# HTDerekLiu/surface_multigrid_code

Measured on AMD Instinct MI355X. Metric: V-cycles/sec + fine-level SpMV GB/s (% HBM peak), 1M-vert mesh fp64, higher is better.
Workload: dtype f64; 1 GPU; C3: bunny_15K_init x3 midpoint subdivision, 1011330 verts, 5 levels, M_bary+0.01(-L), fp64; n_verts=1011330, nnz=7079298, levels=5, smoother=gs, rhs_columns_per_gpu=1, parallelism=single GPU

## Files before the change

surface_multigrid_code_amd/csrc/smg_cycle.cpp:

```cpp
#include <hip/hip_runtime.h>

#include <algorithm>
#include <chrono>
#include <cmath>
#include <cstdarg>
#include <cstdio>
#include <cstdlib>
#include <cstring>
#include <functional>
#include <memory>
#include <numeric>
#include <string>
#include <thread>
#include <vector>

#include "smg_internal.hpp"

using namespace smg;


static hipError_t ensure_map(DevBuf<int>& d, const std::vector<int>& host)
{
    if (d.n == host.size() && (d.p || host.empty())) return hipSuccess;
    return d.upload(host);
// ... 360 lines not shown
    }
    if (k > h->kcap32) {
        drop_graphs(h);
        for (int lv = 0; lv < L; lv++) {
            Level& Lv = h->lv[lv];
            const size_t rows = (lv == L - 1) ? (size_t)h->nc_pad : (size_t)Lv.n;
            HIPCHK(Lv.b32.alloc(rows * k));
            HIPCHK(Lv.u32.alloc(rows * k));
            HIPCHK(hipMemsetAsync(Lv.b32.p, 0, rows * k * sizeof(float), h->stream));
            HIPCHK(hipMemsetAsync(Lv.u32.p, 0, rows * k * sizeof(float), h->stream));
            if (lv < L - 1) HIPCHK(Lv.r32.alloc(rows * k));
            Lv.t32.release(); Lv.d32.release();
        }
        h->kcap32 = k;
    }
    for (int lv = 0; lv < L - 1; lv++) {
        Level& Lv = h->lv[lv];
        if (level_is_jacobi(h, lv) && Lv.t32.n < (size_t)Lv.n * h->kcap32) {
            drop_graphs(h);
            HIPCHK(Lv.t32.alloc((size_t)Lv.n * h->kcap32));
            HIPCHK(hipMemsetAsync(Lv.t32.p, 0, (size_t)Lv.n * h->kcap32 * sizeof(float), h->stream));
        }
        if (level_kind(h, lv) == LV_CHEBY && Lv.d32.n < (size_t)Lv.n * h->kcap32) {
            drop_graphs(h);
            HIPCHK(Lv.d32.alloc((size_t)Lv.n * h->kcap32));
            HIPCHK(hipMemsetAsync(Lv.d32.p, 0, (size_t)Lv.n * h->kcap32 * sizeof(float), h->stream));
        }
    }
    if (h->coarse_schur) {
        const size_t need = (size_t)h->sch.view.ns_pad * std::max(h->kcap32, 1);
        if (h->sch.g32.n < need || h->sch.xs32.n < need) {
            drop_graphs(h);
            HIPCHK(h->sch.g32.alloc(need));
            HIPCHK(h->sch.xs32.alloc(need));
            HIPCHK(hipMemsetAsync(h->sch.g32.p, 0, need * sizeof(float), h->stream));
            HIPCHK(hipMemsetAsync(h->sch.xs32.p, 0, need * sizeof(float), h->stream));
        }
        h->sch.view.g32 = h->sch.g32.p; h->sch.view.xs32 = h->sch.xs32.p;
    }
    return SMG_OK;
}

int smg::level_kind(const smg_hierarchy* h, int lv)
{
    if (lv < 0 || lv >= h->n_levels - 1) return LV_GS;
    switch (h->smoother) {
        case SMG_SMOOTH_JACOBI: return LV_JACOBI;
        case SMG_SMOOTH_HYBRID: return h->lv[lv].n <= h->jacobi_max_rows ? LV_JACOBI : LV_GS;
        case SMG_SMOOTH_CHEBYSHEV: return LV_CHEBY;
        case SMG_SMOOTH_HYBRID_CHEBYSHEV: return h->lv[lv].n <= h->jacobi_max_rows ? LV_CHEBY : LV_GS;
    }
    return LV_GS;
}

struct ChebyCoef { double c1, c2; };
static void cheby_coefs(double lam, double frac, int degree, std::vector<ChebyCoef>& out)
{
    out.resize((size_t)std::max(degree, 0));
    const double lmax = lam, lmin = lam * frac;
    const double theta = (lmax + lmin) / 2.0, delta = (lmax - lmin) / 2.0;
    const double sigma = theta / delta;
    double rho = 1.0 / sigma;
    for (int s = 0; s < degree; s++) {
        if (s == 0) { out[s].c1 = 0.0; out[s].c2 = 1.0 / theta; }
        else {
            const double rho_new = 1.0 / (2.0 * sigma - rho);
            out[s].c1 = rho_new * rho;
            out[s].c2 = 2.0 * rho_new / delta;
            rho = rho_new;
        }
    }
}

template <typename T> struct Prec;
static inline int coarse_cols(const smg_hierarchy* h, int k) { return (h->coarse_cols > 0 && h->coarse_cols < k) ? h->coarse_cols : k; }

template <> struct Prec<double> {
    static double* b(Level& L) { return L.b.p; }
    static double* u(Level& L) { return L.u.p; }
    static double* r(Level& L) { return L.r.p; }
    static double* t(Level& L) { return L.t.p; }
    static double* d(Level& L) { return L.d.p; }
    static void set_d(FirstColour& fc, Level& L) { fc.d = L.d.p; }
    static const SellDev& A(Level& L) { return L.dA.view; }
    static const SellDev& G(Level& L) { return L.gs_on_transpose ? L.dAT.view : L.dA.view; }
    static const SellDev& P(Level& L) { return L.dP.view; }
    static const SellDev& PT(Level& L) { return L.dPT.view; }
    static bool has_vals(const SellDev& V) { return V.val != nullptr; }
    static hipError_t sell(SellMode m, const SellDev& V, int s0, int s1, const double* x, const double* bb, double* y, int k, const Ctrl* ctrl,
                           hipStream_t st, double* zero_rows = nullptr, const FirstColour* first = nullptr, double omega = 1.0)
    { return launch_sell(m, V, s0, s1, x, bb, y, k, ctrl, nullptr, nullptr, st, zero_rows, first, omega); }
    static hipError_t coarse(smg_hierarchy* h, Level& L, int k, const Ctrl* ctrl)
    {
        if (h->union_m > 0) return launch_blockdiag_gemv_add(h->un.view, h->d_Ainv.p, h->nc, L.b.p, L.u.p, k, ctrl, h->stream);
        if (h->coarse_sparse) return launch_sparse_coarse_solve(h->c_view, L.b.p, L.u.p, k, ctrl, h->stream);
        if (h->coarse_schur) return launch_schur_solve(h->sch.view, L.b.p, L.u.p, k, ctrl, h->stream);
        return launch_dense_gemv_add(h->d_Ainv.p, h->nc, h->nc_pad, L.b.p, L.u.p, coarse_cols(h, k), k, ctrl, h->stream, h->d_sympart.p);
    }
    static hipError_t opA(smg_hierarchy* h, Level& L, bool smoother_image, SellMode m, int s0, int s1, const double* x, const double* bb, double* y, int k,
                          const Ctrl* ctrl, const FirstColour* fc = nullptr, double omega = 1.0)
    {
        if (h->bs == 3) {
            const Bsr3Dev& V = (smoother_image && L.gs_on_transpose) ? L.bAT.view : L.bA.view;
            return launch_bsr3(m, V, s0, s1 < 0 ? V.n_slices : s1, x, bb, y, k, ctrl, nullptr, nullptr, h->stream, omega, fc ? fc->c1 : 0.0, fc ? fc->d : nullptr);
        }
        const SellDev& V = smoother_image ? G(L) : A(L);
        return sell(m, V, s0, s1 < 0 ? V.n_slices : s1, x, bb, y, k, ctrl, h->stream, nullptr, fc, omega);
    }
};
template <> struct Prec<float> {
    static float* b(Level& L) { return L.b32.p; }
    static float* u(Level& L) { return L.u32.p; }
    static float* r(Level& L) { return L.r32.p; }
    static float* t(Level& L) { return L.t32.p; }
    static float* d(Level& L) { return L.d32.p; }
    static void set_d(FirstColour& fc, Level& L) { fc.df = L.d32.p; }
    static const SellDev& A(Level& L) { return L.dA32; }
    static const SellDev& G(Level& L) { return L.gs_on_transpose ? L.dAT32 : L.dA32; }
    static const SellDev& P(Level& L) { return L.dP32; }
    static const SellDev& PT(Level& L) { return L.dPT32; }
    static bool has_vals(const SellDev& V) { return V.valf != nullptr; }
    static hipError_t sell(SellMode m, const SellDev& V, int s0, int s1, const float* x, const float* bb, float* y, int k, const Ctrl* ctrl,
                           hipStream_t st, float* zero_rows = nullptr, const FirstColour* first = nullptr, double omega = 1.0)
    { return launch_sell_f32(m, V, s0, s1, x, bb, y, k, ctrl, st, zero_rows, first, omega); }
    static hipError_t coarse(smg_hierarchy* h, Level& L, int k, const Ctrl* ctrl)
    {
        if (h->coarse_schur) return launch_schur_solve_f32(h->sch.view, L.b32.p, L.u32.p, k, ctrl, h->stream);
        return launch_dense_gemv_add_f32(h->d_Ainv32.p, h->nc, h->nc_pad, L.b32.p, L.u32.p, coarse_cols(h, k), k, ctrl, h->stream, (float*)h->d_sympart.p);
    }
    static hipError_t opA(smg_hierarchy* h, Level& L, bool smoother_image, SellMode m, int s0, int s1, const float* x, const float* bb, float* y, int k,
                          const Ctrl* ctrl, const FirstColour* fc = nullptr, double omega = 1.0)
    {
        if (h->bs == 3) {
            const Bsr3Dev& V = (smoother_image && L.gs_on_transpose) ? L.bAT.view : L.bA.view;
            return launch_bsr3_f32(m, V, s0, s1 < 0 ? V.n_slices : s1, x, bb, y, k, ctrl, h->stream, omega, fc ? fc->c1 : 0.0, fc ? fc->df : nullptr);
        }
        const SellDev& V = smoother_image ? G(L) : A(L);
        return sell(m, V, s0, s1 < 0 ? V.n_slices : s1, x, bb, y, k, ctrl, h->stream, nullptr, fc, omega);
    }
};

static const std::vector<int>& colour_slices(const smg_hierarchy* h, const Level& Lv)
{
    if (h->bs == 3) return (Lv.gs_on_transpose ? Lv.bAT : Lv.bA).color_slice_ptr;
    return (Lv.gs_on_transpose ? Lv.dAT : Lv.dA).color_slice_ptr;
}

enum { FIRST_NONE = 0,
       FIRST_LAUNCH = 1,
       FIRST_SWEEP = 2 };

template <typename T>
static int enqueue_gs(smg_hierarchy* h, int lv, const T* b, T* u, int k, int iters, const Ctrl* ctrl, int first = FIRST_NONE, T* t = nullptr)
{
    Level& Lv = h->lv[lv];
    ProfGuard pg(h, "MG: relaxation");
    if (std::is_same<T, double>::value && first == FIRST_NONE) {
        if (const WgsBuf* W = wgs_plan(h, lv, k)) {
            for (int it = 0; it < iters; it++)
                for (size_t c = 0; c + 1 < W->color_ptr.size(); c++)
                    HIPCHK(launch_wgs(W->view, W->color_ptr[c], W->color_ptr[c + 1], (const double*)b, (double*)u, k, ctrl, h->stream));
            return SMG_OK;
        }
        if (const BgsBuf* Q = bgs_plan(h, lv, k)) {
            for (int it = 0; it < iters; it++)
                for (size_t c = 0; c + 1 < Q->color_ptr.size(); c++)
                    HIPCHK(launch_bgs(Q->view, Q->color_ptr[c], Q->color_ptr[c + 1], (const double*)b, (double*)u, k, ctrl, h->stream));
            return SMG_OK;
        }
    }
    const std::vector<int>& cs = colour_slices(h, Lv);
    for (int it = first == FIRST_SWEEP ? 1 : 0; it < iters; it++)
        for (size_t c = (it == 0 && first == FIRST_LAUNCH) ? 1 : 0; c + 1 < cs.size(); c++) {
            if (it == 1 && first == FIRST_SWEEP) HIPCHK(Prec<T>::sell(SELL_GS_OOP, Prec<T>::G(Lv), cs[c], cs[c + 1], t, b, u, k, ctrl, h->stream));
            else HIPCHK(Prec<T>::opA(h, Lv, true, SELL_GS, cs[c], cs[c + 1], u, b, u, k, ctrl));
        }
    return SMG_OK;
}

static int enqueue_gs_tiled(smg_hierarchy* h, int lv, const TiledDev& plan, const double* b, double* const buf[2], int* cur, int k, const Ctrl* ctrl)
{
    ProfGuard pg(h, "MG: relaxation");
    HIPCHK(launch_tiled_gs(plan, buf[*cur], b, buf[1 - *cur], k, ctrl, h->stream));
    *cur ^= 1;
    return SMG_OK;
}
template <typename T> static const TiledDev* tiled_for(const smg_hierarchy*, Level&, int, int, int) { return nullptr; }
template <> const TiledDev* tiled_for<double>(const smg_hierarchy* h, Level& Lv, int lv, int k, int sweeps)
{
    const TiledDev* p = tiled_plan(h, lv, k, sweeps);
    return (p && Lv.t.p) ? p : nullptr;
}
template <typename T> static int enqueue_gs_tiled_t(smg_hierarchy*, int, const TiledDev&, const T*, T* const*, int*, int, const Ctrl*) { return SMG_ERR_INVALID; }
template <> int enqueue_gs_tiled_t<double>(smg_hierarchy* h, int lv, const TiledDev& plan, const double* b, double* const* buf, int* cur, int k, const Ctrl* ctrl)
{
    double* const two[2] = {buf[0], buf[1]};
    return enqueue_gs_tiled(h, lv, plan, b, two, cur, k, ctrl);
}

template <typename T>
static int enqueue_jacobi(smg_hierarchy* h, int lv, const T* b, T* const buf[2], int* cur, int k, int iters, const Ctrl* ctrl)
{
    Level& Lv = h->lv[lv];
    ProfGuard pg(h, "MG: relaxation");
    for (int it = 0; it < iters; it++) {
        HIPCHK(Prec<T>::opA(h, Lv, true, SELL_JACOBI, 0, -1, buf[*cur], b, buf[1 - *cur], k, ctrl, nullptr, h->omega));
        *cur ^= 1;
    }
    return SMG_OK;
}

template <typename T>
static int enqueue_cheby(smg_hierarchy* h, int lv, const T* b, T* const buf[2], int* cur, int k, int iters, const Ctrl* ctrl, bool first_done = false)
{
    if (iters <= 0) return SMG_OK;
    Level& Lv = h->lv[lv];
    ProfGuard pg(h, "MG: relaxation");
    std::vector<ChebyCoef> cf;
    cheby_coefs(Lv.lam, h->cheby_fraction, iters + 1, cf);
    for (int s = first_done ? 1 : 0; s <= iters; s++) {
        FirstColour fc;
        Prec<T>::set_d(fc, Lv);
        fc.c1 = cf[s].c1;
        HIPCHK(Prec<T>::opA(h, Lv, true, SELL_CHEBY, 0, -1, buf[*cur], b, buf[1 - *cur], k, ctrl, &fc, cf[s].c2));
        *cur ^= 1;
    }
    return SMG_OK;
}

static bool fuse_first_colour() { static const int on = env_int("SMG_FUSE_FIRST", 1); return on != 0; }

template <typename T>
static int enqueue_vcycle_t(smg_hierarchy* h, int lv, int k, int pre, int post, const Ctrl* ctrl, int first = FIRST_NONE)
{
    const bool first_done = first != FIRST_NONE;
    const int L = h->n_levels;
    Level& Lv = h->lv[lv];
    if (lv == L - 1) {
        ProfGuard pg(h, "MG: coarse solve");
        HIPCHK(Prec<T>::coarse(h, Lv, k, ctrl));
        return SMG_OK;
    }
    Level& Lc = h->lv[lv + 1];
    const int kind = level_kind(h, lv);
    const bool jac = kind != LV_GS;
    T* const buf[2] = {Prec<T>::u(Lv), Prec<T>::t(Lv)};
    int cur = 0;
    const TiledDev* tl_pre = (kind == LV_GS && pre > 0 && first != FIRST_SWEEP) ? tiled_for<T>(h, Lv, lv, k, pre) : nullptr;
    const TiledDev* tl_post = (kind == LV_GS && post > 0) ? tiled_for<T>(h, Lv, lv, k, post) : nullptr;
    int rc;
    if (kind == LV_JACOBI) {
        if (first_done) cur = 1;
        rc = enqueue_jacobi<T>(h, lv, Prec<T>::b(Lv), buf, &cur, k, pre - (first_done ? 1 : 0), ctrl);
    } else if (kind == LV_CHEBY) {
        if (first_done) cur = 1;
        rc = enqueue_cheby<T>(h, lv, Prec<T>::b(Lv), buf, &cur, k, pre, ctrl, first_done);
    } else if (tl_pre) rc = enqueue_gs_tiled_t<T>(h, lv, *tl_pre, Prec<T>::b(Lv), buf, &cur, k, ctrl);
    else rc = enqueue_gs<T>(h, lv, Prec<T>::b(Lv), buf[0], k, pre, ctrl, first, buf[1]);
    if (rc) return rc;
    {
        ProfGuard pg(h, "MG: residual");
        HIPCHK(Prec<T>::opA(h, Lv, false, SELL_RESID, 0, -1, buf[cur], Prec<T>::b(Lv), Prec<T>::r(Lv), k, ctrl));
    }
    const SellBuf& Gc = Lc.gs_on_transpose ? Lc.dAT : Lc.dA;
    const int kind_c = level_kind(h, lv + 1);
    const bool jac_c = kind_c != LV_GS;
    const bool tiled_c = level_kind(h, lv + 1) == LV_GS && pre > 0 && tiled_for<T>(h, Lc, lv + 1, k, pre) != nullptr;
    const bool fuse = h->bs == 1 && !tiled_c && !(std::is_same<T, double>::value && (bgs_plan(h, lv + 1, k) || wgs_plan(h, lv + 1, k))) && fuse_first_colour() && lv + 1 < L - 1 && pre > 0 && Prec<T>::has_vals(Prec<T>::G(Lc)) && (jac_c ? Gc.n_all > 0 : Gc.n_first > 0);
    const int kt = k * h->bs;
    {
        ProfGuard pg(h, "MG: restrict");
        FirstColour fc;
        if (fuse) {
            fc.diag_slot = Gc.diag_slot.p; fc.n_first = jac_c ? Gc.n_all : Gc.n_first;
            fc.val = Prec<T>::G(Lc).val; fc.valf = Prec<T>::G(Lc).valf;
            fc.jacobi = kind_c == LV_CHEBY ? 2 : (jac_c ? 1 : 0); fc.omega = h->omega;
            if (kind_c == LV_CHEBY) {
                std::vector<ChebyCoef> cf;
                cheby_coefs(Lc.lam, h->cheby_fraction, 1, cf);
                fc.omega = cf[0].c2;
                Prec<T>::set_d(fc, Lc);
            }
        }
        T* init = (fuse && jac_c) ? Prec<T>::t(Lc) : Prec<T>::u(Lc);
        HIPCHK(Prec<T>::sell(SELL_AX, Prec<T>::PT(Lc), 0, Prec<T>::PT(Lc).n_slices, Prec<T>::r(Lv), nullptr, Prec<T>::b(Lc), kt, ctrl, h->stream, init,
                             fuse ? &fc : nullptr));
    }
    rc = enqueue_vcycle_t<T>(h, lv + 1, k, pre, post, ctrl, fuse ? FIRST_LAUNCH : FIRST_NONE);
    if (rc) return rc;
    {
        ProfGuard pg(h, "MG: prolong");
        int dst = cur;
        const int flips = tl_post ? 1 : kind == LV_CHEBY ? (post > 0 ? post + 1 : 0) : post;
        if ((jac || tl_post) && ((cur + flips) & 1)) dst = 1 - cur;
        if (!jac && !tl_post && cur == 1) dst = 0;
        HIPCHK(Prec<T>::sell(SELL_ADD, Prec<T>::P(Lc), 0, Prec<T>::P(Lc).n_slices, Prec<T>::u(Lc), buf[cur], buf[dst], kt, ctrl, h->stream));
        cur = dst;
    }
    if (kind == LV_CHEBY) return enqueue_cheby<T>(h, lv, Prec<T>::b(Lv), buf, &cur, k, post, ctrl);
    if (jac) return enqueue_jacobi<T>(h, lv, Prec<T>::b(Lv), buf, &cur, k, post, ctrl);
    if (tl_post) return enqueue_gs_tiled_t<T>(h, lv, *tl_post, Prec<T>::b(Lv), buf, &cur, k, ctrl);
    return enqueue_gs<T>(h, lv, Prec<T>::b(Lv), buf[0], k, post, ctrl);
}

static int enqueue_vcycle(smg_hierarchy* h, int lv, int k, int pre, int post, const Ctrl* ctrl, int first = FIRST_NONE)
{
    return enqueue_vcycle_t<double>(h, lv, k, pre, post, ctrl, first);
}
static int enqueue_vcycle32(smg_hierarchy* h, int lv, int k, int pre, int post, const Ctrl* ctrl)
{
    return enqueue_vcycle_t<float>(h, lv, k, pre, post, ctrl);
}

static int enqueue_relax(smg_hierarchy* h, int lv, const double* b, double* u, int k, int iters, const Ctrl* ctrl)
{
    if (!level_is_jacobi(h, lv)) {
        Level& Lg = h->lv[lv];
        if (const TiledDev* tl = tiled_for<double>(h, Lg, lv, k, iters)) {
            double* const two[2] = {u, Lg.t.p};
            int c2 = 0;
            int rc = enqueue_gs_tiled(h, lv, *tl, b, two, &c2, k, ctrl);
            if (rc) return rc;
            HIPCHK(hipMemcpyAsync(u, Lg.t.p, (size_t)Lg.n * k * sizeof(double), hipMemcpyDeviceToDevice, h->stream));
            return SMG_OK;
        }
        return enqueue_gs<double>(h, lv, b, u, k, iters, ctrl);
    }
    Level& Lv = h->lv[lv];
    double* const buf[2] = {u, Lv.t.p};
    int cur = 0;
    int rc = level_kind(h, lv) == LV_CHEBY ? enqueue_cheby<double>(h, lv, b, buf, &cur, k, iters, ctrl)
                                           : enqueue_jacobi<double>(h, lv, b, buf, &cur, k, iters, ctrl);
    if (rc) return rc;
    if (cur == 1) HIPCHK(hipMemcpyAsync(u, Lv.t.p, (size_t)Lv.n * k * sizeof(double), hipMemcpyDeviceToDevice, h->stream));
    return SMG_OK;
}

static bool head_fusable(smg_hierarchy* h, int k)
{
    static const int on = env_int("SMG_FUSE_HEAD", 1);
    if (!on || h->precision != 0 || h->n_levels < 2 || h->prof_on || h->bs != 1 || h->union_m > 0) return false;
    Level& L0 = h->lv[0];
    if (L0.gs_on_transpose) return false;
    if (bgs_plan(h, 0, k) || wgs_plan(h, 0, k)) return false;
    if (level_kind(h, 0) == LV_GS && tiled_plan(h, 0, k, h->pre) && L0.t.p) return false;
// ... 900 lines not shown
```

surface_multigrid_code_amd/csrc/smg_device.hip:

```cpp
#include <hip/hip_runtime.h>

#include <cstdlib>
#include <type_traits>

#include "smg_device.hpp"
#include "smg_device_inl.hpp"
#include "smg_gj_inl.hpp"

namespace smg {


__device__ int g_never_done = 0;
const int* never_done()
{
    static const int* p = nullptr;
    if (!p) { void* q = nullptr; if (hipGetSymbolAddress(&q, HIP_SYMBOL(g_never_done)) == hipSuccess) p = (const int*)q; }
    return p;
}


template <typename T> struct CoarseInit { T* u; const T* gs_val; const int* diag_slot; int n_first; int jacobi; T omega; T* d; T c1; };

template <int MODE, int KB, typename T, int W0C = -1, int WPB = 4>
__global__ __launch_bounds__(64 * WPB) void k_sell(const int* a_col, const T* a_val, const int* a_order, const int* a_slice_off, int a_stride,
                                              int a_w_lo, int s_begin, int s_end, int n_blocks, int use_order, const T* x,
                                              const int* a_slice_row, const int* a_slice_w, const T* b, T* y, int ld, const int* done,
                                              double* partials, CoarseInit<T> z)
{
    struct { const int *slice_row, *slice_off, *slice_w, *order, *col; int stride, w_lo; } A = {a_slice_row, a_slice_off, a_slice_w, a_order,
                                                                                               a_col, a_stride, a_w_lo};
    constexpr int C = 64;
    const int lane = threadIdx.x & 63;
    const int wave = threadIdx.x >> 6;
    constexpr int wpb = WPB;
    constexpr bool GS = sell_is_gs(MODE), OOP = sell_is_oop(MODE), JAC = sell_is_jacobi(MODE), CHEB = sell_is_cheby(MODE), HEAD = sell_is_head(MODE);
    int bid;
    if (GS && n_blocks < 0) { if (blockIdx.x & 7) return; bid = blockIdx.x >> 3; }
    else bid = xcd_remap(blockIdx.x, n_blocks);
    const int ls = __builtin_amdgcn_readfirstlane(s_begin + bid * wpb + wave);
    double ss = 0.0;
    int stop = 0;
    if (ls < s_end) {
        const int s = (!GS && use_order) ? A.order[ls] : ls;
        const int W0 = W0C >= 0 ? W0C : (A.w_lo < 8 ? A.w_lo : 8);
        const int off0 = (W0C >= 0 || A.stride) ? s * A.stride : A.slice_off[s];
        const int* cp = A.col + (size_t)off0 * C + lane;
        const T* vp = a_val + (size_t)off0 * C + lane;
        constexpr int U = W0C > 8 ? W0C : 8;
        int c0[U];
        T v0[U];
#pragma unroll
        for (int t = 0; t < U; t++) {
            if (t < W0) { c0[t] = cp[(size_t)t * C]; v0[t] = vp[(size_t)t * C]; }
            else { c0[t] = -1; v0[t] = (T)0; }
        }
        {
            size_t keep = (size_t)x ^ (size_t)A.slice_row ^ (size_t)A.slice_w ^ (size_t)b ^ (size_t)y ^ (size_t)done ^ (size_t)ld;
            if (MODE == SELL_AX) keep ^= (size_t)z.u ^ (size_t)z.gs_val ^ (size_t)z.diag_slot ^ (size_t)z.n_first ^ (size_t)z.jacobi ^ (size_t)z.d;
            if (CHEB) keep ^= (size_t)z.d;
            asm("" : "+s"(keep));
            if (keep == 0x5a5a5a5a5a5a5a5bull) return;
        }
        stop = load_flag(done);
        const int row0 = A.slice_row[s];
        const int nrow = A.slice_row[s + 1] - row0;
        const int w = A.slice_w[s];
        const int rowb = row0 + lane;
        const int split = OOP ? A.slice_row[s_begin] : 0;
        T acc[KB];
        T accr[KB];
        T diag = (T)1;
        T xi[KB];
        T dold[KB];
        T bv[KB];
        const bool live = lane < nrow;
        T zd = (T)1;
        if (MODE == SELL_AX && live && rowb < z.n_first) zd = z.gs_val[z.diag_slot[rowb]];
#pragma unroll
        for (int q = 0; q < KB; q++) {
            acc[q] = (T)0; accr[q] = (T)0; xi[q] = (T)0; dold[q] = (T)0;
            if (MODE == SELL_AX) bv[q] = (T)0;
            else bv[q] = live ? b[(size_t)rowb * ld + q] : (T)0;
            if (CHEB && live && z.c1 != (T)0) dold[q] = z.d[(size_t)rowb * ld + q];
        }
        auto consume = [&](const int (&c)[U], const T (&v)[U]) {
            T xv[U][KB];
            T xo[MODE == SELL_GS_HEAD ? U : 1][KB];
#pragma unroll
            for (int t = 0; t < U; t++) {
                const bool use = (c[t] >= 0) && !(GS && c[t] == rowb);
                if constexpr (MODE == SELL_GS_HEAD) {
                    gather_kb<KB, T>(x + (size_t)c[t] * ld, c[t] >= 0, xo[t]);
                    gather_kb<KB, T>((const T*)y + (size_t)c[t] * ld, use && c[t] < split, xv[t]);
                } else if constexpr (MODE == SELL_GS_OOP) {
                    gather_kb<KB, T>((c[t] < split ? (const T*)y : x) + (size_t)c[t] * ld, use, xv[t]);
                } else {
                    gather_kb<KB, T>(x + (size_t)c[t] * ld, use, xv[t]);
                }
            }
#pragma unroll
            for (int t = 0; t < U; t++) {
                if (c[t] >= 0) {
                    if (HEAD) {
#pragma unroll
                        for (int q = 0; q < KB; q++) accr[q] += v[t] * (MODE == SELL_GS_HEAD ? xo[t][q] : xv[t][q]);
                    }
                    if (GS && c[t] == rowb) {
                        diag = v[t];
                    } else if ((JAC || CHEB) && c[t] == rowb) {
                        diag = v[t];
#pragma unroll
                        for (int q = 0; q < KB; q++) xi[q] = xv[t][q];
                    } else {
#pragma unroll
                        for (int q = 0; q < KB; q++) acc[q] += v[t] * ((MODE == SELL_GS_HEAD && c[t] >= split) ? xo[t][q] : xv[t][q]);
                    }
                }
            }
        };
        if (W0 > 0) consume(c0, v0);
        for (int j0 = W0; j0 < w; j0 += U) {
            int c[U];
            T v[U];
#pragma unroll
            for (int t = 0; t < U; t++) {
                if ((j0 + t) < w) { c[t] = cp[(size_t)(j0 + t) * C]; v[t] = vp[(size_t)(j0 + t) * C]; }
                else { c[t] = -1; v[t] = (T)0; }
            }
            consume(c, v);
        }
        if (live && !stop) {
            const size_t o = (size_t)rowb * ld;
#pragma unroll
            for (int q = 0; q < KB; q++) {
                if (MODE == SELL_AX) {
                    y[o + q] = acc[q];
                    if (z.u) {
                        const T t = acc[q] / zd;
                        if (z.jacobi == 2) { const T dn = z.omega * (t - (T)0); z.u[o + q] = (T)0 + dn; z.d[o + q] = dn; }
                        else z.u[o + q] = rowb < z.n_first ? (z.jacobi ? (T)0 + z.omega * (t - (T)0) : t) : (T)0;
                    }
                }
                else if (MODE == SELL_RESID) y[o + q] = bv[q] - acc[q];
                else if (MODE == SELL_ADD) y[o + q] = bv[q] + acc[q];
                else if (GS) y[o + q] = (bv[q] - acc[q]) / diag;
                else if (JAC) { const T t = (bv[q] - acc[q]) / diag; y[o + q] = xi[q] + z.omega * (t - xi[q]); }
                else if (CHEB) {
                    const T t = (bv[q] - acc[q]) / diag;
                    const T r = t - xi[q];
                    const T dn = z.c1 != (T)0 ? z.c1 * dold[q] + z.omega * r : z.omega * r;
                    y[o + q] = xi[q] + dn;
                    z.d[o + q] = dn;
                }
                else { const double t = (double)(bv[q] - acc[q]); ss += t * t; if (MODE == SELL_RESID_BOTH) y[o + q] = bv[q] - acc[q]; }
                if (HEAD) { const double t = (double)(bv[q] - accr[q]); ss += t * t; }
            }
        }
    }
    if (sell_has_ss(MODE)) {
        __shared__ double red[16];
#pragma unroll
        for (int o = 32; o > 0; o >>= 1) ss += __shfl_down(ss, o, 64);
        if (lane == 0) red[wave] = ss;
        __syncthreads();
        if (threadIdx.x == 0 && !stop) {
            double t = 0.0;
            for (int i2 = 0; i2 < wpb; i2++) t += red[i2];
            partials[HEAD ? bid : (int)blockIdx.x] = t;
        }
    }
}

template <int MODE, int KB, int NBMAX>
__global__ __launch_bounds__(256) void k_sell_deep(const int* a_col, const double* a_val, const int* a_order, const int* a_slice_off, int a_stride, int s_begin, int s_end,
                                                   int n_blocks, int use_order, const double* x, const int* a_slice_row, const int* a_slice_w, const double* b, double* y, int ld,
                                                   const int* done, CoarseInit<double> z)
{
    constexpr int C = 64, S = NBMAX * 8;
    const int lane = threadIdx.x & 63, wave = threadIdx.x >> 6;
    const int bid = xcd_remap(blockIdx.x, n_blocks);
    const int ls = __builtin_amdgcn_readfirstlane(s_begin + bid * 4 + wave);
    if (ls >= s_end) return;
    const int s = use_order ? a_order[ls] : ls;
    const int stop = load_flag(done);
    const int oz = __builtin_amdgcn_mbcnt_lo(~0u, 0u) >> 6;
    const int row0 = a_slice_row[s + oz], nrow = a_slice_row[s + 1 + oz] - row0, w = a_slice_w[s + oz];
    const int off0 = a_stride ? s * a_stride : a_slice_off[s + oz];
    const int rowb = row0 + lane;
    const bool live = lane < nrow;
    const int* cp = a_col + (size_t)off0 * C + lane;
    const double* vp = a_val + (size_t)off0 * C + lane;
    int c[S];
    double v[S];
#pragma unroll
    for (int bt = 0; bt < NBMAX; bt++) {
        if (bt * 8 < w) {
#pragma unroll
            for (int t = bt * 8; t < bt * 8 + 8; t++) {
                const int tt = t < w ? t : w - 1;
                c[t] = cp[(size_t)tt * C];
                v[t] = vp[(size_t)tt * C];
            }
        } else {
#pragma unroll
            for (int t = bt * 8; t < bt * 8 + 8; t++) { c[t] = -1; v[t] = 0.0; }
        }
    }
    double zd = 1.0, bv[KB];
    if (MODE == SELL_AX && live && rowb < z.n_first) zd = z.gs_val[z.diag_slot[rowb]];
#pragma unroll
    for (int q = 0; q < KB; q++) bv[q] = (MODE == SELL_RESID && live) ? b[(size_t)rowb * ld + q] : 0.0;
    double xv[S][KB];
#pragma unroll
    for (int t = 0; t < S; t++) {
        const bool use = c[t] >= 0 && t < w;
        if (!use) v[t] = 0.0;
        gather_kb<KB, double>(x + (size_t)(use ? c[t] : 0) * ld, use, xv[t]);
    }
    double acc[KB];
#pragma unroll
    for (int q = 0; q < KB; q++) acc[q] = 0.0;
#pragma unroll
    for (int bt = 0; bt < NBMAX; bt++) {
        if (bt * 8 < w) {
#pragma unroll
            for (int t = bt * 8; t < bt * 8 + 8; t++)
#pragma unroll
                for (int q = 0; q < KB; q++) acc[q] += v[t] * xv[t][q];
        }
    }
    if (live && !stop) {
        const size_t o = (size_t)rowb * ld;
#pragma unroll
        for (int q = 0; q < KB; q++) {
            if (MODE == SELL_AX) {
                y[o + q] = acc[q];
                if (z.u) {
                    const double t = acc[q] / zd;
                    if (z.jacobi == 2) { const double dn = z.omega * (t - 0.0); z.u[o + q] = 0.0 + dn; z.d[o + q] = dn; }
                    else z.u[o + q] = rowb < z.n_first ? (z.jacobi ? 0.0 + z.omega * (t - 0.0) : t) : 0.0;
                }
            } else y[o + q] = bv[q] - acc[q];
        }
    }
}
static bool deep_wanted(int mode, int w_max, int kb)
{
    static const int on = getenv("SMG_DEEP") ? atoi(getenv("SMG_DEEP")) : 1;
    static const int wmin = getenv("SMG_DEEP_MIN_W") ? atoi(getenv("SMG_DEEP_MIN_W")) : 13;
    if (!on || (mode != SELL_AX && mode != SELL_RESID) || w_max < wmin || w_max > 64) return false;
    const int nbm = w_max <= 24 ? 3 : w_max <= 40 ? 5 : 8;
    return nbm == 3 ? kb <= 3 : nbm == 5 ? kb <= 2 : kb == 1;
}

template <int MODE, int KW, typename T, int R = 2, int U = 8>
__global__ __launch_bounds__(256) void k_sell_wide(const int* a_col, const T* a_val, const int* a_order, const int* a_slice_off, int a_stride,
                                                   int s_begin, int s_end, int n_blocks, int use_order, const T* x,
                                                   const int* a_slice_row, const int* a_slice_w, const T* b, T* y, int ld,
                                                   const int* done, double* partials, CoarseInit<T> z)
{
    struct { const int *slice_row, *slice_off, *slice_w, *order, *col; int stride; } A = {a_slice_row, a_slice_off, a_slice_w, a_order, a_col,
                                                                                        a_stride};
    constexpr bool GS = sell_is_gs(MODE), OOP = sell_is_oop(MODE), JAC = sell_is_jacobi(MODE), CHEB = sell_is_cheby(MODE), HEAD = sell_is_head(MODE);
    const int stop = load_flag(done);
    constexpr int G = 64 / KW;
    constexpr int RW = R * G;
// ... 123 lines not shown
    }
}

template <typename T>
__global__ __launch_bounds__(256) void k_long_ax(const int* rows, const int* ptr, const int* col, const T* val, int nl, const T* x, T* y, int ld, int k,
                                                 const int* done, CoarseInit<T> z)
{
    const int stop = load_flag(done);
    const int lane = threadIdx.x & 63;
    const long wid = (long)blockIdx.x * 4 + (threadIdx.x >> 6);
    if (wid >= (long)nl * k) return;
    const int r = (int)(wid / k), c = (int)(wid % k);
    const int row = rows[r], p0 = ptr[r], p1 = ptr[r + 1];
    T zd = (T)1;
    if (z.u && row < z.n_first) zd = z.gs_val[z.diag_slot[row]];
    T acc = (T)0;
    for (int base = p0; base < p1; base += 64) {
        const int t = base + lane;
        T prod = (T)0;
        if (t < p1) prod = val[t] * x[(size_t)col[t] * ld + c];
        const int n = (p1 - base) < 64 ? (p1 - base) : 64;
        for (int i = 0; i < n; i++) acc += __shfl(prod, i, 64);
    }
    if (lane == 0 && !stop) {
        const size_t o = (size_t)row * ld + c;
        y[o] = acc;
        if (z.u) {
            const T t = acc / zd;
            if (z.jacobi == 2) { const T dn = z.omega * (t - (T)0); z.u[o] = (T)0 + dn; z.d[o] = dn; }
            else z.u[o] = row < z.n_first ? (z.jacobi ? (T)0 + z.omega * (t - (T)0) : t) : (T)0;
        }
    }
}
template <typename T>
__global__ __launch_bounds__(256) void k_long_ax_cols(const int* rows, const int* ptr, const int* col, const T* val, int nl, const T* x, T* y, int ld, int k,
                                                      const int* done, CoarseInit<T> z)
{
    const int stop = load_flag(done);
    const int lane = threadIdx.x & 63;
    const int cblocks = (k + 63) >> 6;
    const long wid = (long)blockIdx.x * 4 + (threadIdx.x >> 6);
    if (wid >= (long)nl * cblocks) return;
    const int r = (int)(wid / cblocks), c = (int)(wid % cblocks) * 64 + lane;
    const bool colok = c < k;
    const int row = rows[r], p0 = ptr[r], p1 = ptr[r + 1];
    T zd = (T)1;
    if (z.u && row < z.n_first) zd = z.gs_val[z.diag_slot[row]];
    T acc = (T)0;
    constexpr int U = 32;
    for (int base = p0; base < p1; base += 64) {
        const int t = base + lane;
        const int ce = t < p1 ? col[t] : 0;
        const T ve = t < p1 ? val[t] : (T)0;
        const int n = (p1 - base) < 64 ? (p1 - base) : 64;
        for (int i0 = 0; i0 < n; i0 += U) {
            T xv[U], vv[U];
#pragma unroll
            for (int i = 0; i < U; i++) {
                const int cc = __shfl(ce, (i0 + i) & 63, 64);
                vv[i] = __shfl(ve, (i0 + i) & 63, 64);
                xv[i] = (i0 + i < n && colok) ? x[(size_t)cc * ld + c] : (T)0;
            }
#pragma unroll
            for (int i = 0; i < U; i++) if (i0 + i < n) acc += vv[i] * xv[i];
        }
    }
    if (colok && !stop) {
        const size_t o = (size_t)row * ld + c;
        y[o] = acc;
        if (z.u) {
            const T t = acc / zd;
            if (z.jacobi == 2) { const T dn = z.omega * (t - (T)0); z.u[o] = (T)0 + dn; z.d[o] = dn; }
            else z.u[o] = row < z.n_first ? (z.jacobi ? (T)0 + z.omega * (t - (T)0) : t) : (T)0;
        }
    }
}
template <typename T> static const T* host_long_vals(const SellDev& A);
template <> const double* host_long_vals<double>(const SellDev& A) { return A.long_val; }
template <> const float* host_long_vals<float>(const SellDev& A) { return A.long_valf; }

template <typename T> static const T* host_vals(const SellDev& A);
template <typename T> static CoarseInit<T> coarse_init(T* zero_rows, int c0, const FirstColour* first, double omega)
{
    CoarseInit<T> z{zero_rows ? zero_rows + c0 : nullptr, nullptr, nullptr, 0, 0, (T)omega, nullptr, (T)0};
    if (first) {
        if constexpr (std::is_same<T, double>::value) z.d = first->d ? first->d + c0 : nullptr; else z.d = first->df ? first->df + c0 : nullptr;
        z.c1 = (T)first->c1;
    }
    if (zero_rows && first && first->n_first > 0) {
        if constexpr (std::is_same<T, double>::value) z.gs_val = first->val; else z.gs_val = first->valf;
        z.diag_slot = first->diag_slot;
        z.n_first = (z.gs_val && z.diag_slot) ? first->n_first : 0;
        z.jacobi = first->jacobi;
        if (first->jacobi) z.omega = (T)first->omega;
    }
    return z;
}
template <> const double* host_vals<double>(const SellDev& A) { return A.val; }
template <> const float* host_vals<float>(const SellDev& A) { return A.valf; }

static long wide_latency_max()
{
    static const long v = getenv("SMG_WIDE_LAT_MAX") ? atol(getenv("SMG_WIDE_LAT_MAX")) : 16384;
    return v;
}
static bool wide_latency_variant(int n_slices, int kw) { return (long)n_slices * kw <= wide_latency_max(); }

template <int MODE, int KW, typename T>
static void launch_wide_one(const SellDev& A, int s_begin, int s_end, int use_order, const T* x, const T* b, T* y,
                            int k, const int* done, double* partials, CoarseInit<T> zero_rows, hipStream_t st, int* nb_out)
{
    const int ns = s_end - s_begin;
    if constexpr (KW < 64) if (wide_latency_variant(ns, KW)) {
        const int nb = (ns * KW + 3) / 4;
#define SMG_WIDE_LAT(UU) hipLaunchKernelGGL((k_sell_wide<MODE, KW, T, 1, UU>), dim3(nb), dim3(256), 0, st, A.col, host_vals<T>(A), A.order, A.slice_off, A.stride, \
                                             s_begin, s_end, nb, use_order, x, A.slice_row, A.slice_w, b, y, k, done, partials, zero_rows)
        if (A.w_max <= 8) SMG_WIDE_LAT(8);
        else if (A.w_max <= 16) SMG_WIDE_LAT(16);
        else SMG_WIDE_LAT(32);
#undef SMG_WIDE_LAT
        *nb_out = nb;
        return;
    }
    const int waves = ns * (KW / 2);
    const int nb = (waves + 3) / 4;
    hipLaunchKernelGGL((k_sell_wide<MODE, KW, T>), dim3(nb), dim3(256), 0, st, A.col, host_vals<T>(A), A.order, A.slice_off, A.stride, s_begin, s_end, nb, use_order, x,
                       A.slice_row, A.slice_w, b, y, k, done, partials, zero_rows);
    *nb_out = nb;
}

int sell_wide_blocks(int n_slices, int k)
{
    int tot = 0, c0 = 0;
    while (k - c0 >= 8) { int kw = 64; while (kw > k - c0) kw >>= 1; tot += (n_slices * kw + 3) / 4; c0 += kw; }
    return tot;
}

static constexpr int sell_wpb() { return 4; }
static int gs_wpb() { static const int v = getenv("SMG_GS_WPB") ? atoi(getenv("SMG_GS_WPB")) : 4; return v; }
int sell_blocks(int n_slices) { return (n_slices + sell_wpb() - 1) / sell_wpb(); }

template <int MODE, typename T>
static hipError_t launch_sell_mode(const SellDev& A, int s_begin, int s_end_in, const T* x, const T* b, T* y,
                                   int k, const Ctrl* ctrl, double* partials, int* n_blocks, hipStream_t st, T* zero_rows, const FirstColour* first,
                                   double omega)
{
    int s_end = s_end_in;
    if (MODE == SELL_ADD && !b) b = y;
    const int ns = s_end - s_begin;
    const int nb = sell_blocks(ns);
    const int* done = ctrl ? &ctrl->done : never_done();
    static const int dbg_empty = getenv("SMG_DEBUG_EMPTY") ? atoi(getenv("SMG_DEBUG_EMPTY")) : 0;
    if (dbg_empty == 1) s_end = s_begin;
    const int use_order = (A.order && s_begin == 0 && s_end == A.n_slices) ? 1 : 0;
    if (n_blocks) *n_blocks = 0;
    if (ns <= 0) return hipSuccess;
    int c0 = 0;
    size_t poff = 0;
    {
        while (k - c0 >= 8) {
            int kw = 64;
            while (kw > k - c0) kw >>= 1;
            const T* xx = x ? x + c0 : nullptr;
            const T* bb = b ? b + c0 : nullptr;
            T* yy = y ? y + c0 : nullptr;
            double* pp = partials ? partials + poff : nullptr;
            const CoarseInit<T> zz = coarse_init<T>(zero_rows, c0, first, omega);
            int wnb = 0;
            switch (kw) {
                case 64: launch_wide_one<MODE, 64, T>(A, s_begin, s_end, use_order, xx, bb, yy, k, done, pp, zz, st, &wnb); break;
                case 32: launch_wide_one<MODE, 32, T>(A, s_begin, s_end, use_order, xx, bb, yy, k, done, pp, zz, st, &wnb); break;
                case 16: launch_wide_one<MODE, 16, T>(A, s_begin, s_end, use_order, xx, bb, yy, k, done, pp, zz, st, &wnb); break;
                default: launch_wide_one<MODE, 8, T>(A, s_begin, s_end, use_order, xx, bb, yy, k, done, pp, zz, st, &wnb); break;
            }
            poff += (size_t)wnb;
            c0 += kw;
        }
    }
    static const int one_xcd_max = getenv("SMG_ONE_XCD_MAX") ? atoi(getenv("SMG_ONE_XCD_MAX")) : 32;
    const bool one_xcd = sell_is_gs(MODE) && nb <= one_xcd_max;
    const int grid = one_xcd ? nb * 8 : nb, nbarg = one_xcd ? -nb : nb;
    for (; c0 < k; c0 += 4) {
        const int kb = (k - c0) < 4 ? (k - c0) : 4;
        const T* xx = x ? x + c0 : nullptr;
        const T* bb = b ? b + c0 : nullptr;
        T* yy = y ? y + c0 : nullptr;
        double* pp = partials ? partials + poff : nullptr;
        const CoarseInit<T> zz = coarse_init<T>(zero_rows, c0, first, omega);
        poff += (size_t)nb;
        if constexpr (std::is_same<T, double>::value && (MODE == SELL_AX || MODE == SELL_RESID)) {
            int kd = kb;
            if (kd == 4 && !deep_wanted(MODE, A.w_max, 4) && deep_wanted(MODE, A.w_max, 2)) kd = 2;
            if (deep_wanted(MODE, A.w_max, kd) || (kd > 1 && deep_wanted(MODE, A.w_max, 1))) {
                for (int cc = 0; cc < kb;) {
                    int kk = kb - cc;
                    while (kk > 1 && !deep_wanted(MODE, A.w_max, kk)) kk--;
                    const int nbm = A.w_max <= 24 ? 3 : A.w_max <= 40 ? 5 : 8;
                    const CoarseInit<T> zc = coarse_init<T>(zero_rows, c0 + cc, first, omega);
#define SMG_DEEP_LAUNCH(KB, NB) hipLaunchKernelGGL((k_sell_deep<MODE, KB, NB>), dim3(nb), dim3(256), 0, st, A.col, A.val, A.order, A.slice_off, A.stride, s_begin, s_end, nb, use_order, \
                                                   xx ? xx + cc : nullptr, A.slice_row, A.slice_w, bb ? bb + cc : nullptr, yy + cc, k, done, zc)
                    if (nbm == 3) { if (kk == 1) SMG_DEEP_LAUNCH(1, 3); else if (kk == 2) SMG_DEEP_LAUNCH(2, 3); else SMG_DEEP_LAUNCH(3, 3); }
                    else if (nbm == 5) { if (kk == 1) SMG_DEEP_LAUNCH(1, 5); else SMG_DEEP_LAUNCH(2, 5); }
                    else SMG_DEEP_LAUNCH(1, 8);
#undef SMG_DEEP_LAUNCH
                    cc += kk;
                }
                continue;
            }
        }
        switch (kb) {
            case 1: {
                const int w0 = A.stride > 0 ? (A.w_lo < 8 ? A.w_lo : 8) : -1;
                static const int pitch_env = getenv("SMG_PITCH_SPEC_MAX") ? atoi(getenv("SMG_PITCH_SPEC_MAX")) : -1;
                const int pitch_max = pitch_env >= 0 ? pitch_env : (sell_is_gs(MODE) ? 32 : 64);
                if (nb <= pitch_max && A.stride == 12 && w0 >= 7) hipLaunchKernelGGL((k_sell<MODE, 1, T, 12>), dim3(grid), dim3(64 * sell_wpb()), 0, st, A.col, host_vals<T>(A), A.order, A.slice_off, A.stride, A.w_lo, s_begin, s_end, nbarg, use_order, xx, A.slice_row, A.slice_w, bb, yy, k, done, pp, zz);
                else if (w0 == 7 && MODE == SELL_GS && !one_xcd && gs_wpb() == 8) hipLaunchKernelGGL((k_sell<MODE == SELL_GS ? MODE : SELL_GS, 1, T, 7, 8>), dim3((ns + 7) / 8), dim3(512), 0, st, A.col, host_vals<T>(A), A.order, A.slice_off, A.stride, A.w_lo, s_begin, s_end, (ns + 7) / 8, use_order, xx, A.slice_row, A.slice_w, bb, yy, k, done, pp, zz);
                else if (w0 == 7 && MODE == SELL_GS && !one_xcd && gs_wpb() == 2) hipLaunchKernelGGL((k_sell<MODE == SELL_GS ? MODE : SELL_GS, 1, T, 7, 2>), dim3((ns + 1) / 2), dim3(128), 0, st, A.col, host_vals<T>(A), A.order, A.slice_off, A.stride, A.w_lo, s_begin, s_end, (ns + 1) / 2, use_order, xx, A.slice_row, A.slice_w, bb, yy, k, done, pp, zz);
                else if (w0 == 7) hipLaunchKernelGGL((k_sell<MODE, 1, T, 7>), dim3(grid), dim3(64 * sell_wpb()), 0, st, A.col, host_vals<T>(A), A.order, A.slice_off, A.stride, A.w_lo, s_begin, s_end, nbarg, use_order, xx, A.slice_row, A.slice_w, bb, yy, k, done, pp, zz);
                else if (w0 == 8) hipLaunchKernelGGL((k_sell<MODE, 1, T, 8>), dim3(grid), dim3(64 * sell_wpb()), 0, st, A.col, host_vals<T>(A), A.order, A.slice_off, A.stride, A.w_lo, s_begin, s_end, nbarg, use_order, xx, A.slice_row, A.slice_w, bb, yy, k, done, pp, zz);
                else if (w0 == 2) hipLaunchKernelGGL((k_sell<MODE, 1, T, 2>), dim3(grid), dim3(64 * sell_wpb()), 0, st, A.col, host_vals<T>(A), A.order, A.slice_off, A.stride, A.w_lo, s_begin, s_end, nbarg, use_order, xx, A.slice_row, A.slice_w, bb, yy, k, done, pp, zz);
                else hipLaunchKernelGGL((k_sell<MODE, 1, T>), dim3(grid), dim3(64 * sell_wpb()), 0, st, A.col, host_vals<T>(A), A.order, A.slice_off, A.stride, A.w_lo, s_begin, s_end, nbarg, use_order, xx, A.slice_row, A.slice_w, bb, yy, k, done, pp, zz);
                break;
            }
            case 2:
                if (A.stride > 0 && A.w_lo == 7) hipLaunchKernelGGL((k_sell<MODE, 2, T, 7>), dim3(grid), dim3(64 * sell_wpb()), 0, st, A.col, host_vals<T>(A), A.order, A.slice_off, A.stride, A.w_lo, s_begin, s_end, nbarg, use_order, xx, A.slice_row, A.slice_w, bb, yy, k, done, pp, zz);
                else hipLaunchKernelGGL((k_sell<MODE, 2, T>), dim3(grid), dim3(64 * sell_wpb()), 0, st, A.col, host_vals<T>(A), A.order, A.slice_off, A.stride, A.w_lo, s_begin, s_end, nbarg, use_order, xx, A.slice_row, A.slice_w, bb, yy, k, done, pp, zz);
                break;
            case 3:
                if (A.stride > 0 && A.w_lo == 7) hipLaunchKernelGGL((k_sell<MODE, 3, T, 7>), dim3(grid), dim3(64 * sell_wpb()), 0, st, A.col, host_vals<T>(A), A.order, A.slice_off, A.stride, A.w_lo, s_begin, s_end, nbarg, use_order, xx, A.slice_row, A.slice_w, bb, yy, k, done, pp, zz);
                else hipLaunchKernelGGL((k_sell<MODE, 3, T>), dim3(grid), dim3(64 * sell_wpb()), 0, st, A.col, host_vals<T>(A), A.order, A.slice_off, A.stride, A.w_lo, s_begin, s_end, nbarg, use_order, xx, A.slice_row, A.slice_w, bb, yy, k, done, pp, zz);
                break;
            default:
                if (A.stride > 0 && A.w_lo == 7) hipLaunchKernelGGL((k_sell<MODE, 4, T, 7>), dim3(grid), dim3(64 * sell_wpb()), 0, st, A.col, host_vals<T>(A), A.order, A.slice_off, A.stride, A.w_lo, s_begin, s_end, nbarg, use_order, xx, A.slice_row, A.slice_w, bb, yy, k, done, pp, zz);
                else hipLaunchKernelGGL((k_sell<MODE, 4, T>), dim3(grid), dim3(64 * sell_wpb()), 0, st, A.col, host_vals<T>(A), A.order, A.slice_off, A.stride, A.w_lo, s_begin, s_end, nbarg, use_order, xx, A.slice_row, A.slice_w, bb, yy, k, done, pp, zz);
                break;
        }
    }
// ... 1234 lines not shown
```

surface_multigrid_code_amd/csrc/smg_device.hpp:

```cpp
#pragma once
#include <hip/hip_runtime_api.h>

#include <cstdint>

namespace smg {

struct Ctrl {
    int done;
    int n_his;
    int status;
    int just_done;
    double sumsq;
    double tol;
    double* r_his;
    int his_cap;
    int pad_;
    double r_last, r_prev;
};

struct SellDev {
    int n_rows = 0, n_cols = 0, n_slices = 0;
    int C = 64;
    const int* slice_row = nullptr;
    const int* slice_off = nullptr;
    const int* slice_w = nullptr;
    int stride = 0;
    int w_lo = 0;
    int w_max = 0;
    const int* order = nullptr;
    const int* col = nullptr;
    const double* val = nullptr;
    const float* valf = nullptr;
    int long_n = 0;
    const int* long_row = nullptr;
    const int* long_ptr = nullptr;
    const int* long_col = nullptr;
    const double* long_val = nullptr;
    const float* long_valf = nullptr;
};

enum SellMode {
    SELL_AX = 0,
    SELL_RESID = 1,
    SELL_RESID_SS = 2,
    SELL_ADD = 3,
    SELL_GS = 4,
    SELL_RESID_BOTH = 5,
    SELL_JACOBI = 6,
    SELL_CHEBY = 7,
    SELL_GS_OOP = 8,
    SELL_GS_HEAD = 9,
    SELL_JACOBI_HEAD = 10,
    SELL_CHEBY_HEAD = 11,
};
constexpr bool sell_is_gs(int m) { return m == SELL_GS || m == SELL_GS_OOP || m == SELL_GS_HEAD; }
constexpr bool sell_is_oop(int m) { return m == SELL_GS_OOP || m == SELL_GS_HEAD; }
constexpr bool sell_is_jacobi(int m) { return m == SELL_JACOBI || m == SELL_JACOBI_HEAD; }
constexpr bool sell_is_cheby(int m) { return m == SELL_CHEBY || m == SELL_CHEBY_HEAD; }
constexpr bool sell_is_head(int m) { return m == SELL_GS_HEAD || m == SELL_JACOBI_HEAD || m == SELL_CHEBY_HEAD; }
constexpr bool sell_has_ss(int m) { return sell_is_head(m) || m == SELL_RESID_SS || m == SELL_RESID_BOTH; }

struct FirstColour {
    const int* diag_slot = nullptr;
    int n_first = 0;
    const double* val = nullptr;
    const float* valf = nullptr;
    int jacobi = 0;
    double omega = 1.0;
    double* d = nullptr;
    float* df = nullptr;
    double c1 = 0.0;
};
hipError_t launch_sell(SellMode mode, const SellDev& A, int s_begin, int s_end, const double* x, const double* b,
                       double* y, int k, const Ctrl* ctrl, double* partials, int* n_blocks, hipStream_t st,
                       double* zero_rows = nullptr, const FirstColour* first = nullptr, double omega = 1.0);
hipError_t launch_sell_f32(SellMode mode, const SellDev& A, int s_begin, int s_end, const float* x, const float* b,
                           float* y, int k, const Ctrl* ctrl, hipStream_t st, float* zero_rows = nullptr,
                           const FirstColour* first = nullptr, double omega = 1.0);
hipError_t launch_gershgorin(const SellDev& A, double* out, hipStream_t st);
struct Bsr3Dev {
    int n_vert = 0, n_slices = 0, w_max = 0;
    const int* slice_row = nullptr;
    const int* slice_off = nullptr;
    const int* slice_w = nullptr;
    const int* order = nullptr;
    const int* col = nullptr;
    const double* val = nullptr;
    const float* valf = nullptr;
};
hipError_t launch_bsr3(SellMode mode, const Bsr3Dev& A, int s_begin, int s_end, const double* x, const double* b, double* y, int k, const Ctrl* ctrl,
                       double* partials, int* n_blocks, hipStream_t st, double omega = 1.0, double c1 = 0.0, double* dvec = nullptr);
hipError_t launch_bsr3_f32(SellMode mode, const Bsr3Dev& A, int s_begin, int s_end, const float* x, const float* b, float* y, int k, const Ctrl* ctrl, hipStream_t st,
                           double omega = 1.0, double c1 = 0.0, float* dvec = nullptr);
hipError_t launch_bsr3_gershgorin(const Bsr3Dev& A, double* out, hipStream_t st);
int bsr3_blocks(int n_slices);
hipError_t launch_bsr3_fill(const int* ptr, const int* col, const double* val, const int* gptr, const int* gcol, const int* perm, const int* iperm, const Bsr3Dev& B,
                            size_t panel_cols, bool transposed, hipStream_t st);

struct BgsDev {
    int n_blocks = 0, n_colors = 0, xrows = 0;
    const int* hdr = nullptr;
    const int* xrow = nullptr;
    const int* ugrow = nullptr;
    const int* ulrow = nullptr;
    const double* udiag = nullptr;
    const int* eidx = nullptr;
    const double* eval = nullptr;
};
hipError_t launch_bgs(const BgsDev& P, int b_begin, int b_end, const double* b, double* u, int k, const Ctrl* ctrl, hipStream_t st);

struct WgsDev {
    int n_pieces = 0, n_colors = 0, rim_pitch = 0, nb_max = 0;
    const int* hdr = nullptr;
    const int* grow = nullptr;
    const int* meta = nullptr;
    const double* diag = nullptr;
    const int* rim = nullptr;
    const unsigned* eoff = nullptr;
    const double* eval = nullptr;
};
hipError_t launch_wgs(const WgsDev& P, int q_begin, int q_end, const double* b, double* u, int k, const Ctrl* ctrl, hipStream_t st);

struct UnionDev {
    int m = 0, his_cap = 0, max_rows = 0;
    const int* rows = nullptr;
    const int* rptr = nullptr;
    const int* crow_member = nullptr;
    const long long* moff = nullptr;
    const int* mlda = nullptr;
    const int* mrow0 = nullptr;
    double* ss = nullptr;
    double* his = nullptr;
    int* nhis = nullptr;
    int* done = nullptr;
    double* zsave = nullptr;
};
hipError_t launch_blockdiag_gemv_add(const UnionDev& U, const double* Ainv, int n, const double* b, double* u, int k, const Ctrl* ctrl, hipStream_t st);
hipError_t launch_union_sumsq_decide(const UnionDev& U, const double* r, const double* u, int k, Ctrl* ctrl, hipStream_t st);
hipError_t launch_union_restore(const UnionDev& U, double* u, int k, const Ctrl* ctrl, hipStream_t st);
hipError_t launch_scatter_dense(double* dense, const double* src, const long long* pos, int nnz, hipStream_t st);
hipError_t launch_dense_identity(double* dense, int np, int n, hipStream_t st);

struct TiledDev {
    int n_tiles = 0, nc = 0, P = 0, sweeps = 0, max_ext = 0, w_max = 0, threads = 512;
    const int* hdr = nullptr;
    const int* ext_rows = nullptr;
    const int* pcol = nullptr;
    const double* pval = nullptr;
    const int* prow = nullptr;
    const double* pdiag = nullptr;
};
hipError_t launch_tiled_gs(const TiledDev& T, const double* x, const double* b, double* y, int k, const Ctrl* ctrl, hipStream_t st);
hipError_t tiled_gs_prepare(int max_ext);

// ... 82 lines not shown
```

Measured before the change: 3324 V-cycles/s.

## Fuse last-colour GS sweep with residual computation for those rows

On the final pre-smoothing sweep, the last colour's Gauss-Seidel kernel now also writes the residual for its rows, since after that update those rows' residual is b - (offdiag + diag*u_new). The following residual SpMV then runs only over the slices of the earlier colours, using a limit on the ordered slice index so reordered launches skip slices belonging to the last colour. This removes one SpMV pass over the last colour's rows per level. In exchange it adds a residual store to the GS kernel and extra order-limit checks in the SELL kernels.

Result: no change. 3313 V-cycles/s, median of 6 (-0.3%).

```diff
diff --git a/surface_multigrid_code_amd/csrc/smg_cycle.cpp b/surface_multigrid_code_amd/csrc/smg_cycle.cpp
--- a/surface_multigrid_code_amd/csrc/smg_cycle.cpp
+++ b/surface_multigrid_code_amd/csrc/smg_cycle.cpp
@@ -466,6 +466,7 @@
     static double* t(Level& L) { return L.t.p; }
     static double* d(Level& L) { return L.d.p; }
     static void set_d(FirstColour& fc, Level& L) { fc.d = L.d.p; }
+    static void set_r(FirstColour& fc, double* r) { fc.r = r; }
     static const SellDev& A(Level& L) { return L.dA.view; }
     static const SellDev& G(Level& L) { return L.gs_on_transpose ? L.dAT.view : L.dA.view; }
     static const SellDev& P(Level& L) { return L.dP.view; }
@@ -499,6 +500,7 @@
     static float* t(Level& L) { return L.t32.p; }
     static float* d(Level& L) { return L.d32.p; }
     static void set_d(FirstColour& fc, Level& L) { fc.df = L.d32.p; }
+    static void set_r(FirstColour& fc, float* r) { fc.rf = r; }
     static const SellDev& A(Level& L) { return L.dA32; }
     static const SellDev& G(Level& L) { return L.gs_on_transpose ? L.dAT32 : L.dA32; }
     static const SellDev& P(Level& L) { return L.dP32; }
@@ -535,7 +537,7 @@
        FIRST_SWEEP = 2 };
 
 template <typename T>
-static int enqueue_gs(smg_hierarchy* h, int lv, const T* b, T* u, int k, int iters, const Ctrl* ctrl, int first = FIRST_NONE, T* t = nullptr)
+static int enqueue_gs(smg_hierarchy* h, int lv, const T* b, T* u, int k, int iters, const Ctrl* ctrl, int first = FIRST_NONE, T* t = nullptr, T* r_last = nullptr)
 {
     Level& Lv = h->lv[lv];
     ProfGuard pg(h, "MG: relaxation");
@@ -554,10 +556,13 @@
         }
     }
     const std::vector<int>& cs = colour_slices(h, Lv);
+    FirstColour fr;
+    Prec<T>::set_r(fr, r_last);
     for (int it = first == FIRST_SWEEP ? 1 : 0; it < iters; it++)
         for (size_t c = (it == 0 && first == FIRST_LAUNCH) ? 1 : 0; c + 1 < cs.size(); c++) {
-            if (it == 1 && first == FIRST_SWEEP) HIPCHK(Prec<T>::sell(SELL_GS_OOP, Prec<T>::G(Lv), cs[c], cs[c + 1], t, b, u, k, ctrl, h->stream));
-            else HIPCHK(Prec<T>::opA(h, Lv, true, SELL_GS, cs[c], cs[c + 1], u, b, u, k, ctrl));
+            const FirstColour* fc = (r_last && it == iters - 1 && c + 2 == cs.size()) ? &fr : nullptr;
+            if (it == 1 && first == FIRST_SWEEP) HIPCHK(Prec<T>::sell(SELL_GS_OOP, Prec<T>::G(Lv), cs[c], cs[c + 1], t, b, u, k, ctrl, h->stream, nullptr, fc));
+            else HIPCHK(Prec<T>::opA(h, Lv, true, SELL_GS, cs[c], cs[c + 1], u, b, u, k, ctrl, fc));
         }
     return SMG_OK;
 }
@@ -615,6 +620,18 @@
 static bool fuse_first_colour() { static const int on = env_int("SMG_FUSE_FIRST", 1); return on != 0; }
 
 template <typename T>
+static bool last_resid_fusable(smg_hierarchy* h, int lv, int k, int pre, int first, bool tiled_pre)
+{
+    static const int on = env_int("SMG_FUSE_LAST_RESID", 1);
+    if (!on || h->bs != 1 || k >= 8 || pre <= 0 || tiled_pre || level_kind(h, lv) != LV_GS) return false;
+    Level& Lv = h->lv[lv];
+    if (Lv.gs_on_transpose) return false;
+    if (std::is_same<T, double>::value && (wgs_plan(h, lv, k) || bgs_plan(h, lv, k))) return false;
+    if (first == FIRST_SWEEP && pre < 2) return false;
+    return colour_slices(h, Lv).size() >= 3;
+}
+
+template <typename T>
 static int enqueue_vcycle_t(smg_hierarchy* h, int lv, int k, int pre, int post, const Ctrl* ctrl, int first = FIRST_NONE)
 {
     const bool first_done = first != FIRST_NONE;
@@ -632,6 +649,7 @@
     int cur = 0;
     const TiledDev* tl_pre = (kind == LV_GS && pre > 0 && first != FIRST_SWEEP) ? tiled_for<T>(h, Lv, lv, k, pre) : nullptr;
     const TiledDev* tl_post = (kind == LV_GS && post > 0) ? tiled_for<T>(h, Lv, lv, k, post) : nullptr;
+    const bool fuse_last = last_resid_fusable<T>(h, lv, k, pre, first, tl_pre != nullptr);
     int rc;
     if (kind == LV_JACOBI) {
         if (first_done) cur = 1;
@@ -640,11 +658,12 @@
         if (first_done) cur = 1;
         rc = enqueue_cheby<T>(h, lv, Prec<T>::b(Lv), buf, &cur, k, pre, ctrl, first_done);
     } else if (tl_pre) rc = enqueue_gs_tiled_t<T>(h, lv, *tl_pre, Prec<T>::b(Lv), buf, &cur, k, ctrl);
-    else rc = enqueue_gs<T>(h, lv, Prec<T>::b(Lv), buf[0], k, pre, ctrl, first, buf[1]);
+    else rc = enqueue_gs<T>(h, lv, Prec<T>::b(Lv), buf[0], k, pre, ctrl, first, buf[1], fuse_last ? Prec<T>::r(Lv) : nullptr);
     if (rc) return rc;
     {
         ProfGuard pg(h, "MG: residual");
-        HIPCHK(Prec<T>::opA(h, Lv, false, SELL_RESID, 0, -1, buf[cur], Prec<T>::b(Lv), Prec<T>::r(Lv), k, ctrl));
+        const int s_end = fuse_last ? colour_slices(h, Lv).end()[-2] : -1;
+        HIPCHK(Prec<T>::opA(h, Lv, false, SELL_RESID, 0, s_end, buf[cur], Prec<T>::b(Lv), Prec<T>::r(Lv), k, ctrl));
     }
     const SellBuf& Gc = Lc.gs_on_transpose ? Lc.dAT : Lc.dA;
     const int kind_c = level_kind(h, lv + 1);
diff --git a/surface_multigrid_code_amd/csrc/smg_device.hip b/surface_multigrid_code_amd/csrc/smg_device.hip
--- a/surface_multigrid_code_amd/csrc/smg_device.hip
+++ b/surface_multigrid_code_amd/csrc/smg_device.hip
@@ -19,7 +19,7 @@
 }
 
 
-template <typename T> struct CoarseInit { T* u; const T* gs_val; const int* diag_slot; int n_first; int jacobi; T omega; T* d; T c1; };
+template <typename T> struct CoarseInit { T* u; const T* gs_val; const int* diag_slot; int n_first; int jacobi; T omega; T* d; T c1; T* r; };
 
 template <int MODE, int KB, typename T, int W0C = -1, int WPB = 4>
 __global__ __launch_bounds__(64 * WPB) void k_sell(const int* a_col, const T* a_val, const int* a_order, const int* a_slice_off, int a_stride,
@@ -40,8 +40,9 @@
     const int ls = __builtin_amdgcn_readfirstlane(s_begin + bid * wpb + wave);
     double ss = 0.0;
     int stop = 0;
-    if (ls < s_end) {
-        const int s = (!GS && use_order) ? A.order[ls] : ls;
+    const int s_sel = (!GS && use_order && ls < s_end) ? A.order[ls] : ls;
+    if (ls < s_end && !(!GS && use_order && s_sel >= use_order)) {
+        const int s = s_sel;
         const int W0 = W0C >= 0 ? W0C : (A.w_lo < 8 ? A.w_lo : 8);
         const int off0 = (W0C >= 0 || A.stride) ? s * A.stride : A.slice_off[s];
         const int* cp = A.col + (size_t)off0 * C + lane;
@@ -58,6 +59,7 @@
             size_t keep = (size_t)x ^ (size_t)A.slice_row ^ (size_t)A.slice_w ^ (size_t)b ^ (size_t)y ^ (size_t)done ^ (size_t)ld;
             if (MODE == SELL_AX) keep ^= (size_t)z.u ^ (size_t)z.gs_val ^ (size_t)z.diag_slot ^ (size_t)z.n_first ^ (size_t)z.jacobi ^ (size_t)z.d;
             if (CHEB) keep ^= (size_t)z.d;
+            if (GS) keep ^= (size_t)z.r;
             asm("" : "+s"(keep));
             if (keep == 0x5a5a5a5a5a5a5a5bull) return;
         }
@@ -143,7 +145,11 @@
                 }
                 else if (MODE == SELL_RESID) y[o + q] = bv[q] - acc[q];
                 else if (MODE == SELL_ADD) y[o + q] = bv[q] + acc[q];
-                else if (GS) y[o + q] = (bv[q] - acc[q]) / diag;
+                else if (GS) {
+                    const T yn = (bv[q] - acc[q]) / diag;
+                    y[o + q] = yn;
+                    if (z.r) z.r[o + q] = bv[q] - (acc[q] + diag * yn);
+                }
                 else if (JAC) { const T t = (bv[q] - acc[q]) / diag; y[o + q] = xi[q] + z.omega * (t - xi[q]); }
                 else if (CHEB) {
                     const T t = (bv[q] - acc[q]) / diag;
@@ -182,6 +188,7 @@
     const int ls = __builtin_amdgcn_readfirstlane(s_begin + bid * 4 + wave);
     if (ls >= s_end) return;
     const int s = use_order ? a_order[ls] : ls;
+    if (use_order && s >= use_order) return;
     const int stop = load_flag(done);
     const int oz = __builtin_amdgcn_mbcnt_lo(~0u, 0u) >> 6;
     const int row0 = a_slice_row[s + oz], nrow = a_slice_row[s + 1 + oz] - row0, w = a_slice_w[s + oz];
@@ -471,10 +478,11 @@
 template <typename T> static const T* host_vals(const SellDev& A);
 template <typename T> static CoarseInit<T> coarse_init(T* zero_rows, int c0, const FirstColour* first, double omega)
 {
-    CoarseInit<T> z{zero_rows ? zero_rows + c0 : nullptr, nullptr, nullptr, 0, 0, (T)omega, nullptr, (T)0};
+    CoarseInit<T> z{zero_rows ? zero_rows + c0 : nullptr, nullptr, nullptr, 0, 0, (T)omega, nullptr, (T)0, nullptr};
     if (first) {
         if constexpr (std::is_same<T, double>::value) z.d = first->d ? first->d + c0 : nullptr; else z.d = first->df ? first->df + c0 : nullptr;
         z.c1 = (T)first->c1;
+        if constexpr (std::is_same<T, double>::value) z.r = first->r ? first->r + c0 : nullptr; else z.r = first->rf ? first->rf + c0 : nullptr;
     }
     if (zero_rows && first && first->n_first > 0) {
         if constexpr (std::is_same<T, double>::value) z.gs_val = first->val; else z.gs_val = first->valf;
@@ -536,12 +544,15 @@
 {
     int s_end = s_end_in;
     if (MODE == SELL_ADD && !b) b = y;
+    if (first && (first->r || first->rf) && (!sell_is_gs(MODE) || MODE == SELL_GS_HEAD || k >= 8)) return hipErrorInvalidValue;
+    int limit = 0;
+    if (!sell_is_gs(MODE) && A.order && s_begin == 0 && s_end > 0 && s_end < A.n_slices && k < 8) { limit = s_end; s_end = A.n_slices; }
     const int ns = s_end - s_begin;
     const int nb = sell_blocks(ns);
     const int* done = ctrl ? &ctrl->done : never_done();
     static const int dbg_empty = getenv("SMG_DEBUG_EMPTY") ? atoi(getenv("SMG_DEBUG_EMPTY")) : 0;
     if (dbg_empty == 1) s_end = s_begin;
-    const int use_order = (A.order && s_begin == 0 && s_end == A.n_slices) ? 1 : 0;
+    const int use_order = (A.order && s_begin == 0 && s_end == A.n_slices) ? (limit ? limit : A.n_slices) : 0;
     if (n_blocks) *n_blocks = 0;
     if (ns <= 0) return hipSuccess;
     int c0 = 0;
diff --git a/surface_multigrid_code_amd/csrc/smg_device.hpp b/surface_multigrid_code_amd/csrc/smg_device.hpp
--- a/surface_multigrid_code_amd/csrc/smg_device.hpp
+++ b/surface_multigrid_code_amd/csrc/smg_device.hpp
@@ -70,6 +70,8 @@
     double* d = nullptr;
     float* df = nullptr;
     double c1 = 0.0;
+    double* r = nullptr;
+    float* rf = nullptr;
 };
 hipError_t launch_sell(SellMode mode, const SellDev& A, int s_begin, int s_end, const double* x, const double* b,
                        double* y, int k, const Ctrl* ctrl, double* partials, int* n_blocks, hipStream_t st,
```
